# radoslawkrolikowski/financial-market-data-analysis

Measured on NVIDIA H100. Metric: sequences/sec (train step) biGRU h=256 seq=128 feat=64, higher is better.
Workload: dtype bf16x3 (fp32-class: split bf16 operand pairs on tensor cores, fp32 accumulate / state / gradients)

## Files before the change

financial_market_data_analysis_b200/csrc/tc_hopper.cuh:

```cuda
#pragma once
#include "common.cuh"
#include "kernels_f32.cuh"
#include <algorithm>
#include <map>
#include <mutex>
#include <cuda.h>
#include <cuda_bf16.h>

namespace htc {

typedef __nv_bfloat16 bf16_t;

__device__ __forceinline__ uint32_t smem_u32(const void* p) { return (uint32_t)__cvta_generic_to_shared(p); }

__device__ __forceinline__ void split_bf16(float x, bf16_t& hi, bf16_t& lo) {
    hi = __float2bfloat16(x);
    lo = __float2bfloat16(x - __bfloat162float(hi));
}

__device__ __forceinline__ void ldsm_x4(uint32_t addr, uint32_t (&r)[4]) {
    asm volatile("ldmatrix.sync.aligned.m8n8.x4.shared.b16 {%0, %1, %2, %3}, [%4];"
                 : "=r"(r[0]), "=r"(r[1]), "=r"(r[2]), "=r"(r[3]) : "r"(addr));
}
__device__ __forceinline__ void ldsm_x2(uint32_t addr, uint32_t (&r)[2]) {
    asm volatile("ldmatrix.sync.aligned.m8n8.x2.shared.b16 {%0, %1}, [%2];" : "=r"(r[0]), "=r"(r[1]) : "r"(addr));
}
__device__ __forceinline__ void mma_bf16(float (&c)[4], const uint32_t (&a)[4], uint32_t b0, uint32_t b1) {
    asm volatile("mma.sync.aligned.m16n8k16.row.col.f32.bf16.bf16.f32 {%0, %1, %2, %3}, {%4, %5, %6, %7}, {%8, %9}, "
                 "{%0, %1, %2, %3};"
                 : "+f"(c[0]), "+f"(c[1]), "+f"(c[2]), "+f"(c[3])
                 : "r"(a[0]), "r"(a[1]), "r"(a[2]), "r"(a[3]), "r"(b0), "r"(b1));
}

template <int PITCH>
__device__ __forceinline__ uint32_t swz(int row, int k) {
    return (uint32_t)(row * PITCH + ((((k >> 3) ^ (row & 7))) << 4) + ((k & 7) << 1));
}

__device__ __forceinline__ uint32_t mapa(uint32_t local_addr, uint32_t cta) {
    uint32_t r;
    asm volatile("mapa.shared::cluster.u32 %0, %1, %2;" : "=r"(r) : "r"(local_addr), "r"(cta));
    return r;
}
__device__ __forceinline__ void st_cluster_v2_f32(uint32_t addr, float2 v) {
    asm volatile("st.shared::cluster.v2.f32 [%0], {%1, %2};" ::"r"(addr), "f"(v.x), "f"(v.y) : "memory");
}
__device__ __forceinline__ void cluster_arrive() { asm volatile("barrier.cluster.arrive.release;" ::: "memory"); }
__device__ __forceinline__ void cluster_wait() { asm volatile("barrier.cluster.wait.acquire;" ::: "memory"); }
__device__ __forceinline__ uint32_t cluster_rank() {
    uint32_t r;
    asm volatile("mov.u32 %0, %%cluster_ctarank;" : "=r"(r));
    return r;
}

constexpr int WG_BM = 128, WG_BN = 128, WG_BK = 64;

__global__ void tc_pack_kernel(const float* __restrict__ src, int64_t s_r, int64_t s_k, int64_t zsrc, int R, int K, int Rp, int Kp,
                               bf16_t* __restrict__ hi, bf16_t* __restrict__ lo) {
    __shared__ float tile[32][33];
    const int z = blockIdx.z, r0 = blockIdx.y * 32, k0 = blockIdx.x * 32;
    const float* a = src + z * zsrc;
    const bool kfast = s_k == 1;
    for (int j = threadIdx.y; j < 32; j += 8) {
        const int r = r0 + (kfast ? j : threadIdx.x), k = k0 + (kfast ? threadIdx.x : j);
        float v = 0.f;
        if (r < R && k < K) v = a[(int64_t)r * s_r + (int64_t)k * s_k];
        if (kfast) tile[j][threadIdx.x] = v; else tile[threadIdx.x][j] = v;
    }
    __syncthreads();
    for (int j = threadIdx.y; j < 32; j += 8) {
        const int r = r0 + j, k = k0 + threadIdx.x;
        const int64_t o = ((int64_t)z * Rp + r) * Kp + k;
        bf16_t h, l;
        split_bf16(tile[j][threadIdx.x], h, l);
        hi[o] = h;
        if (lo) lo[o] = l;
    }
}

__global__ void to_planes_kernel(const float* __restrict__ src, int64_t rows, int cols, int pitch, bf16_t* __restrict__ hi,
                                 bf16_t* __restrict__ lo) {
    const int64_t n = rows * cols;
    for (int64_t i = (int64_t)blockIdx.x * blockDim.x + threadIdx.x; i < n; i += (int64_t)gridDim.x * blockDim.x) {
        const int64_t r = i / cols, c = i % cols, o = r * pitch + c;
        bf16_t h, l;
        split_bf16(src[i], h, l);
        hi[o] = h;
        if (lo) lo[o] = l;
    }
}

__device__ __forceinline__ void mbar_init(uint64_t* bar, uint32_t count) {
    asm volatile("mbarrier.init.shared::cta.b64 [%0], %1;" ::"r"(smem_u32(bar)), "r"(count) : "memory");
}
__device__ __forceinline__ void mbar_arrive_expect_tx(uint64_t* bar, uint32_t bytes) {
    asm volatile("mbarrier.arrive.expect_tx.shared::cta.b64 _, [%0], %1;" ::"r"(smem_u32(bar)), "r"(bytes) : "memory");
}
__device__ __forceinline__ void mbar_arrive(uint64_t* bar) {
    asm volatile("mbarrier.arrive.shared::cta.b64 _, [%0];" ::"r"(smem_u32(bar)) : "memory");
}
__device__ __forceinline__ bool mbar_try_wait(uint64_t* bar, uint32_t parity) {
    uint32_t ok;
    asm volatile(
        "{\n\t.reg .pred p;\n\t"
        "mbarrier.try_wait.parity.shared::cta.b64 p, [%1], %2;\n\t"
        "selp.u32 %0, 1, 0, p;\n\t}" : "=r"(ok) : "r"(smem_u32(bar)), "r"(parity) : "memory");
    return ok != 0;
}
__device__ __forceinline__ bool mbar_try_wait_cluster(uint64_t* bar, uint32_t parity) {
    uint32_t ok;
    asm volatile(
        "{\n\t.reg .pred p;\n\t"
        "mbarrier.try_wait.parity.acquire.cluster.shared::cta.b64 p, [%1], %2;\n\t"
        "selp.u32 %0, 1, 0, p;\n\t}" : "=r"(ok) : "r"(smem_u32(bar)), "r"(parity) : "memory");
    return ok != 0;
}
template <bool CLUSTER = false>
__device__ __forceinline__ void mbar_wait(uint64_t* bar, uint32_t parity) {
    auto ready = [&] { return CLUSTER ? mbar_try_wait_cluster(bar, parity) : mbar_try_wait(bar, parity); };
    if (ready()) return;
    uint64_t t0, t;
    asm volatile("mov.u64 %0, %%globaltimer;" : "=l"(t0));
    for (uint32_t i = 0;; ++i) {
        if (ready()) return;
        if ((i & 1023u) == 1023u) {
            asm volatile("mov.u64 %0, %%globaltimer;" : "=l"(t));
            if (t - t0 > 5000000000ull) __trap();
        }
    }
}
__device__ __forceinline__ void bulk_copy_to_peer(uint32_t src, uint32_t bytes, uint64_t* bar, uint32_t cta) {
    asm volatile("cp.async.bulk.shared::cluster.shared::cta.mbarrier::complete_tx::bytes [%0], [%1], %2, [%3];"
                 ::"r"(mapa(src, cta)), "r"(src), "r"(bytes), "r"(mapa(smem_u32(bar), cta)) : "memory");
}
__device__ __forceinline__ void tma_load_3d(uint32_t dst, const CUtensorMap* m, uint64_t* bar, int c0, int c1, int c2) {
    asm volatile("cp.async.bulk.tensor.3d.shared::cluster.global.mbarrier::complete_tx::bytes [%0], [%1, {%3, %4, %5}], [%2];"
                 ::"r"(dst), "l"(reinterpret_cast<uint64_t>(m)), "r"(smem_u32(bar)), "r"(c0), "r"(c1), "r"(c2) : "memory");
}
__device__ __forceinline__ uint64_t wg_desc(uint32_t saddr, uint32_t lbo) {
    return (uint64_t)((saddr & 0x3FFFF) >> 4) | ((uint64_t)(lbo >> 4) << 16) | ((uint64_t)(1024 >> 4) << 32) | ((uint64_t)1 << 62);
}
template <int TA, int TB>
__device__ __forceinline__ void wgmma_m64n128k16(float (&d)[64], uint64_t da, uint64_t db) {
    asm volatile("wgmma.mma_async.sync.aligned.m64n128k16.f32.bf16.bf16 {%0, %1, %2, %3, %4, %5, %6, %7, %8, %9, %10, %11, %12, %13, %14, %15, %16, %17, %18, %19, %20, %21, %22, %23, %24, %25, %26, %27, %28, %29, %30, %31, %32, %33, %34, %35, %36, %37, %38, %39, %40, %41, %42, %43, %44, %45, %46, %47, %48, %49, %50, %51, %52, %53, %54, %55, %56, %57, %58, %59, %60, %61, %62, %63}, %64, %65, 1, 1, 1, %66, %67;"
                 : "+f"(d[0]), "+f"(d[1]), "+f"(d[2]), "+f"(d[3]), "+f"(d[4]), "+f"(d[5]), "+f"(d[6]), "+f"(d[7]), "+f"(d[8]), "+f"(d[9]), "+f"(d[10]), "+f"(d[11]), "+f"(d[12]), "+f"(d[13]), "+f"(d[14]), "+f"(d[15]), "+f"(d[16]), "+f"(d[17]), "+f"(d[18]), "+f"(d[19]), "+f"(d[20]), "+f"(d[21]), "+f"(d[22]), "+f"(d[23]), "+f"(d[24]), "+f"(d[25]), "+f"(d[26]), "+f"(d[27]), "+f"(d[28]), "+f"(d[29]), "+f"(d[30]), "+f"(d[31]), "+f"(d[32]), "+f"(d[33]), "+f"(d[34]), "+f"(d[35]), "+f"(d[36]), "+f"(d[37]), "+f"(d[38]), "+f"(d[39]), "+f"(d[40]), "+f"(d[41]), "+f"(d[42]), "+f"(d[43]), "+f"(d[44]), "+f"(d[45]), "+f"(d[46]), "+f"(d[47]), "+f"(d[48]), "+f"(d[49]), "+f"(d[50]), "+f"(d[51]), "+f"(d[52]), "+f"(d[53]), "+f"(d[54]), "+f"(d[55]), "+f"(d[56]), "+f"(d[57]), "+f"(d[58]), "+f"(d[59]), "+f"(d[60]), "+f"(d[61]), "+f"(d[62]), "+f"(d[63])
                 : "l"(da), "l"(db), "n"(TA), "n"(TB));
}

struct WgOp {
    int zsel, coff, kshift[2];
};
struct WgJob {
    WgOp a, b;
    float* C; const float* bias; float* part;
    int M, N, tm, tn, batch, splits;
    int kblocks, kbd;
    int kcat;
    int beta;
    int64_t ldc, zC, zBias;
};

template <int NS, int STAGES, int AMN, int BMN>
__global__ void __launch_bounds__(384, 1)
wg_gemm_kernel(const __grid_constant__ CUtensorMap ta_hi, const __grid_constant__ CUtensorMap ta_lo,
               const __grid_constant__ CUtensorMap tb_hi, const __grid_constant__ CUtensorMap tb_lo, const WgJob j) {
    constexpr int NH = NS == 1 ? 1 : 2;
    constexpr int PLANE = WG_BM * WG_BK * 2;
    constexpr int STAGE = 2 * NH * PLANE;
    extern __shared__ __align__(1024) uint8_t wg_smem_raw[];
    uint8_t* sm = reinterpret_cast<uint8_t*>((reinterpret_cast<uintptr_t>(wg_smem_raw) + 1023) & ~(uintptr_t)1023);
    uint64_t* full = reinterpret_cast<uint64_t*>(sm + STAGES * STAGE);
    uint64_t* empty = full + STAGES;
    const int wgi = threadIdx.x / 128, tid = threadIdx.x % 128;
    const int units = j.tm * j.tn * j.batch * j.splits;
    const int per = (j.kblocks + j.splits - 1) / j.splits;
    if (threadIdx.x == 0) {
        for (int i = 0; i < STAGES; ++i) { mbar_init(full + i, 1); mbar_init(empty + i, 2); }
        asm volatile("fence.mbarrier_init.release.cluster;" ::: "memory");
    }
    __syncthreads();
    auto decode = [&](int u, int& s, int& zb, int& m0, int& n0) {
        s = u % j.splits; u /= j.splits;
        n0 = (u % j.tn) * WG_BN; u /= j.tn;
        m0 = (u % j.tm) * WG_BM; zb = u / j.tm;
    };

    if (wgi == 0) {
        if (tid == 0) {
            uint32_t it = 0;
            for (int u = blockIdx.x; u < units; u += gridDim.x) {
                int s, zb, m0, n0;
                decode(u, s, zb, m0, n0);
                const int kb1 = min(j.kblocks, (s + 1) * per);
                for (int kb = s * per; kb < kb1; ++kb, ++it) {
                    const int st = it % STAGES;
                    if (it >= STAGES) mbar_wait(empty + st, ((it / STAGES) - 1) & 1);
                    const uint32_t base = smem_u32(sm + st * STAGE);
                    mbar_arrive_expect_tx(full + st, STAGE);
                    const int dz = j.kcat ? kb / j.kbd : zb, kc = (j.kcat ? kb % j.kbd : kb) * WG_BK;
#pragma unroll
                    for (int h = 0; h < NH; ++h) {
                        const CUtensorMap* ma = h ? &ta_lo : &ta_hi;
                        const CUtensorMap* mb = h ? &tb_lo : &tb_hi;
                        const uint32_t da = base + h * PLANE, db = base + (NH + h) * PLANE;
                        if (AMN) {
                            const int k = kc + (dz ? j.a.kshift[1] : j.a.kshift[0]), r = m0 + dz * j.a.coff;
                            tma_load_3d(da, ma, full + st, r, k, dz * j.a.zsel);
                            tma_load_3d(da + PLANE / 2, ma, full + st, r + 64, k, dz * j.a.zsel);
                        } else {
                            tma_load_3d(da, ma, full + st, kc, m0, dz * j.a.zsel);
                        }
                        if (BMN) {
                            const int k = kc + (dz ? j.b.kshift[1] : j.b.kshift[0]), r = n0 + dz * j.b.coff;
                            tma_load_3d(db, mb, full + st, r, k, dz * j.b.zsel);
                            tma_load_3d(db + PLANE / 2, mb, full + st, r + 64, k, dz * j.b.zsel);
                        } else {
                            tma_load_3d(db, mb, full + st, kc, n0, dz * j.b.zsel);
                        }
                    }
                }
            }
        }
        return;
    }
    const int cg = wgi - 1;
    const int w = tid / 32, l = tid % 32;
    constexpr uint32_t AKS = AMN ? 2048 : 32, BKS = BMN ? 2048 : 32;
    constexpr uint32_t ALBO = AMN ? PLANE / 2 : 16, BLBO = BMN ? PLANE / 2 : 16;
    uint32_t it = 0;
    for (int u = blockIdx.x; u < units; u += gridDim.x) {
        int s, zb, m0, n0;
        decode(u, s, zb, m0, n0);
        const int kb1 = min(j.kblocks, (s + 1) * per);
        float d[64];
#pragma unroll
        for (int i = 0; i < 64; ++i) d[i] = 0.f;
        int prev = -1;
        for (int kb = s * per; kb < kb1; ++kb, ++it) {
            const int st = it % STAGES;
            mbar_wait(full + st, (it / STAGES) & 1);
            const uint32_t base = smem_u32(sm + st * STAGE);
            const uint32_t a_hi = base + cg * (PLANE / 2), a_lo = a_hi + PLANE;
            const uint32_t b_hi = base + NH * PLANE, b_lo = b_hi + PLANE;
            asm volatile("wgmma.fence.sync.aligned;" ::: "memory");
#pragma unroll
            for (int ks = 0; ks < WG_BK / 16; ++ks) {
                wgmma_m64n128k16<AMN, BMN>(d, wg_desc(a_hi + ks * AKS, ALBO), wg_desc(b_hi + ks * BKS, BLBO));
                if (NS != 1) {
                    wgmma_m64n128k16<AMN, BMN>(d, wg_desc(a_hi + ks * AKS, ALBO), wg_desc(b_lo + ks * BKS, BLBO));
                    wgmma_m64n128k16<AMN, BMN>(d, wg_desc(a_lo + ks * AKS, ALBO), wg_desc(b_hi + ks * BKS, BLBO));
                }
            }
            asm volatile("wgmma.commit_group.sync.aligned;" ::: "memory");
            asm volatile("wgmma.wait_group.sync.aligned 1;" ::: "memory");
            if (prev >= 0 && tid == 0) mbar_arrive(empty + prev);
            prev = st;
        }
        asm volatile("wgmma.wait_group.sync.aligned 0;" ::: "memory");
        if (prev >= 0 && tid == 0) mbar_arrive(empty + prev);
        float* C;
        int64_t ldc;
        const float* bias = nullptr;
        if (j.splits > 1) {
            C = j.part + ((int64_t)s * j.batch + zb) * j.M * j.N;
            ldc = j.N;
        } else {
            C = j.C + zb * j.zC;
            ldc = j.ldc;
            if (j.bias) bias = j.bias + zb * j.zBias;
        }
#pragma unroll
        for (int i = 0; i < 16; ++i)
#pragma unroll
            for (int e = 0; e < 4; ++e) {
                const int gm = m0 + cg * 64 + w * 16 + (l >> 2) + (e >= 2 ? 8 : 0);
                const int gn = n0 + 8 * i + 2 * (l & 3) + (e & 1);
                if (gm >= j.M || gn >= j.N) continue;
                float v = d[4 * i + e];
                if (bias) v += bias[gn];
                float* c = C + (int64_t)gm * ldc + gn;
                if (j.beta && j.splits == 1) *c += v;
                else *c = v;
            }
    }
}

__global__ void splitk_reduce_kernel(const float* __restrict__ part, int splits, int batch, int M, int N, float* __restrict__ C,
                                     int64_t ldc, int64_t zC, int beta) {
    const int64_t per = (int64_t)M * N, n = per * batch;
    for (int64_t i = (int64_t)blockIdx.x * blockDim.x + threadIdx.x; i < n; i += (int64_t)gridDim.x * blockDim.x) {
        float v = 0.f;
        for (int s = 0; s < splits; ++s) v += part[(int64_t)s * n + i];
        const int64_t z = i / per, r = i % per;
        float* c = C + z * zC + (r / N) * ldc + r % N;
        *c = beta ? *c + v : v;
    }
}

constexpr int SCAN_U = 64, SCAN_NB = 16, SCAN_THREADS = 256;
constexpr int SCAN_Y = 1, SCAN_G = 2, SCAN_PLANES = 4;
constexpr int SCAN_TRAIN = SCAN_Y | SCAN_G | SCAN_PLANES, SCAN_INFER_LOWER = SCAN_PLANES, SCAN_INFER_TOP = SCAN_Y;

template <int H, int NS>
struct FwdSmem {
    static constexpr int NH = NS == 1 ? 1 : 2;
    static constexpr int NBMAX = NS == 1 ? SCAN_NB : 2 * SCAN_NB;
    static constexpr int NBUF = NBMAX == SCAN_NB ? 2 : 1;
    static constexpr int WP = H * 2;
    static constexpr int WBYTES = 3 * SCAN_U * WP;
    static constexpr int HBYTES = NBMAX * H * 2;
    static constexpr int SLICE = NBMAX * SCAN_U * 2;
    static constexpr int TOTAL = NH * WBYTES + NBUF * NH * HBYTES + 2 * 8;
};

__device__ __forceinline__ void scan_tile(int q, int m2, int ntd, int D, int& d, int& bt0, int& nb) {
    if (q < D * m2) {
        d = q / m2; bt0 = (q % m2) * 2 * SCAN_NB; nb = 2 * SCAN_NB;
    } else {
        const int r = q - D * m2, o = ntd - 2 * m2;
        d = r / o; bt0 = (2 * m2 + r % o) * SCAN_NB; nb = SCAN_NB;
    }
}

template <int NBMAX>
__device__ __forceinline__ uint32_t hsw(int b, int k) {
    return (uint32_t)((k / SCAN_U) * (NBMAX * SCAN_U * 2)) + swz<SCAN_U * 2>(b, k % SCAN_U);
}

__device__ __forceinline__ void mbar_arrive_peer(uint64_t* bar, uint32_t cta) {
    asm volatile("mbarrier.arrive.release.cluster.shared::cluster.b64 _, [%0];" ::"r"(mapa(smem_u32(bar), cta)) : "memory");
}

template <int H, int NS, int OUT, bool LEN, int JN, bool RD = false>
__device__ __forceinline__ void gru_scan_fwd_tile(const float* __restrict__ gi, const float* __restrict__ Whh,
                                                  const float* __restrict__ bhh, int64_t zW, const float* __restrict__ h0,
                                                  float* __restrict__ Y, float* __restrict__ G, float* __restrict__ hn_out,
                                                  bf16_t* __restrict__ yh, bf16_t* __restrict__ yl, int B, int T, int D,
                                                  const int* __restrict__ lens, int d, int bt0,
                                                  const float* __restrict__ mask = nullptr) {
    using S = FwdSmem<H, NS>;
    constexpr int U = SCAN_U, CS = H / U, NH = S::NH, JMAX = JN, jn = JN, nb = JN * SCAN_NB;
    constexpr int NBMAX = nb, NBUF = S::NBUF * S::NBMAX / nb;
    constexpr int HBYTES = nb * H * 2, SLICE = nb * U * 2;
    static_assert(NBUF * HBYTES == S::NBUF * S::HBYTES, "both tile sizes fill the h region");
    static_assert(SCAN_THREADS % (nb * (U / 8)) == 0, "a thread copies the same Y plane row in every pass");
    extern __shared__ __align__(128) uint8_t smem[];
    uint8_t* Wsm = smem;
    uint8_t* Hsm = smem + NH * S::WBYTES;
    uint64_t* full = reinterpret_cast<uint64_t*>(Hsm + NBUF * NH * HBYTES);
    uint64_t* empty = full + 1;
    const int c = (int)cluster_rank();
    const int tid = threadIdx.x, lane = tid & 31, warp = tid >> 5;
    const float* W = Whh + d * zW;

    for (int i = tid; i < 3 * U * H; i += SCAN_THREADS) {
        const int q = i / H, k = i % H, gte = q / U, u = q % U;
        const float v = W[(int64_t)(gte * H + c * U + u) * H + k];
        bf16_t hi, lo;
        split_bf16(v, hi, lo);
        *reinterpret_cast<bf16_t*>(Wsm + swz<S::WP>(q, k)) = hi;
        if (NH == 2) *reinterpret_cast<bf16_t*>(Wsm + S::WBYTES + swz<S::WP>(q, k)) = lo;
    }
    for (int i = tid; i < nb * H; i += SCAN_THREADS) {
        const int b = i / H, k = i % H;
        float v = h0 ? h0[((int64_t)d * B + bt0 + b) * H + k] : 0.f;
        if constexpr (RD) v *= mask[((int64_t)d * B + bt0 + b) * H + k];
        bf16_t hi, lo;
        split_bf16(v, hi, lo);
        *reinterpret_cast<bf16_t*>(Hsm + hsw<NBMAX>(b, k)) = hi;
        if (NH == 2) *reinterpret_cast<bf16_t*>(Hsm + HBYTES + hsw<NBMAX>(b, k)) = lo;
    }
    if (tid == 0) {
        mbar_init(full, 1);
        mbar_init(full + 1, NBUF == 2 ? 1 : CS - 1);
        asm volatile("fence.mbarrier_init.release.cluster;" ::: "memory");
    }

    const int ug = warp >> 1, nt = warp & 1;
    int unit[2], bcol[JMAX][2];
    unit[0] = ug * 16 + (lane >> 2); unit[1] = unit[0] + 8;
#pragma unroll
    for (int j = 0; j < JMAX; ++j) {
        bcol[j][0] = (nt * jn + j) * 8 + 2 * (lane & 3); bcol[j][1] = bcol[j][0] + 1;
    }
    float bias[3][2], hp[JMAX][4], mk[RD ? JMAX : 1][4];
#pragma unroll
    for (int gte = 0; gte < 3; ++gte)
#pragma unroll
        for (int i = 0; i < 2; ++i) bias[gte][i] = bhh[d * zW + gte * H + c * U + unit[i]];
    int len[JMAX][2], rlen = T;
#pragma unroll
    for (int j = 0; j < JMAX; ++j) {
#pragma unroll
        for (int e = 0; e < 4; ++e) {
            const int b = bt0 + bcol[j][e & 1], k = c * U + unit[e >> 1];
            hp[j][e] = h0 ? h0[((int64_t)d * B + b) * H + k] : 0.f;
            if constexpr (RD) mk[j][e] = mask[((int64_t)d * B + b) * H + k];
        }
        len[j][0] = len[j][1] = T;
        if (LEN) { len[j][0] = lens[bt0 + bcol[j][0]]; len[j][1] = lens[bt0 + bcol[j][1]]; }
    }
    if (LEN) rlen = lens[bt0 + (tid / (U / 8)) % nb];
    cluster_arrive();
    cluster_wait();

    const int DH = D * H;
    for (int s = 0; s < T; ++s) {
        const int t = d == 0 ? s : T - 1 - s;
        const int buf = NBUF == 2 ? s & 1 : 0, nbuf = NBUF == 2 ? buf ^ 1 : 0;
        if (s > 0) mbar_wait<true>(full + buf, (NBUF == 2 ? (s - 1) >> 1 : s - 1) & 1);
        if (tid == 0 && s + 1 < T) mbar_arrive_expect_tx(full + nbuf, (CS - 1) * NH * nb * U * 2);
        float giv[3][JMAX][4];
#pragma unroll
        for (int j = 0; j < JMAX; ++j)
#pragma unroll
            for (int e = 0; e < 4; ++e) {
                const int64_t row = (int64_t)(bt0 + bcol[j][e & 1]) * T + t;
                const float* gr = gi + ((int64_t)d * B * T + row) * 3 * H + c * U + unit[e >> 1];
#pragma unroll
                for (int gte = 0; gte < 3; ++gte) giv[gte][j][e] = gr[gte * H];
            }
        float acc[3][JMAX][4];
#pragma unroll
        for (int gte = 0; gte < 3; ++gte)
#pragma unroll
            for (int j = 0; j < JMAX; ++j)
#pragma unroll
                for (int e = 0; e < 4; ++e) acc[gte][j][e] = 0.f;
        const uint32_t hbase = smem_u32(Hsm + buf * NH * HBYTES);
        const uint32_t wbase = smem_u32(Wsm);
#pragma unroll 4
        for (int ks = 0; ks < H / 16; ++ks) {
            uint32_t bh[JMAX][NH][2];
            const int bk = ks * 16 + ((lane >> 3) & 1) * 8;
#pragma unroll
            for (int j = 0; j < JMAX; ++j)
#pragma unroll
// ... 190 lines not shown
                if constexpr (RD) v = LEN && (d == 0 ? t + 1 : t - 1) >= plen[i] ? v : mk[i] * v;
                dhr[i] = v;
            }
        }
        cluster_arrive();
        __syncthreads();
#pragma unroll
        for (int i = 0; i < PAIRS; ++i) {
            const int p = tid + i * SCAN_THREADS, u = p % U, bl = p / U, b = bt0 + bl, j = c * U + u;
            const int64_t row = (int64_t)b * T + t;
            const float r = gr[i], z = gz[i], n = gn[i], hnv = ghn[i], hpv = hprev[i];
            const float dh = dhr[i] + dyv[i];
            float dan = dh * (1.f - z) * (1.f - n * n);
            float dar = dan * hnv * r * (1.f - r);
            float daz = dh * (hpv - n) * z * (1.f - z);
            float dgn = dan * r;
            const bool pad = LEN && t >= plen[i];
            if (pad) dan = dar = daz = dgn = 0.f;
            float* a = dgi + ((int64_t)d * B * T + row) * 3 * H + j;
            float* cg = dgh + ((int64_t)d * B * T + row) * 3 * H + j;
            a[0] = dar; a[H] = daz; a[2 * H] = dan;
            cg[0] = dar; cg[H] = daz; cg[2 * H] = dgn;
            dhz[i] = pad ? dhr[i] : dh * z;
            const float gv[3] = {dar, daz, dgn};
#pragma unroll
            for (int gte = 0; gte < 3; ++gte) {
                bf16_t hi, lo;
                split_bf16(gv[gte], hi, lo);
                *reinterpret_cast<bf16_t*>(Dsm + swz<S::WP>(bl, gte * U + u)) = hi;
                if (NH == 2) *reinterpret_cast<bf16_t*>(Dsm + S::DBYTES + swz<S::WP>(bl, gte * U + u)) = lo;
            }
            bf16_t hi, lo;
            split_bf16(dan, hi, lo);
            const int64_t po = ((int64_t)d * B * T + row) * 3 * H + 2 * H + j;
            gih[po] = hi;
            if (NH == 2) gil[po] = lo;
        }
        if (NS == 1 && s + 1 < T) load_step(s + 1);
        __syncthreads();
        for (int i = tid; i < NH * NR * (Q / 8); i += SCAN_THREADS) {
            const int h = i / (NR * Q / 8), r = (i / (Q / 8)) % NR, q = (i % (Q / 8)) * 8, gte = q / U;
            uint4 v = *reinterpret_cast<const uint4*>(Dsm + h * S::DBYTES + swz<S::WP>(r, q));
            const int64_t o = ((int64_t)d * B * T + (int64_t)(bt0 + r) * T + t) * 3 * H + gte * H + c * U + q % U;
            if (gte < 2) *reinterpret_cast<uint4*>((h ? gil : gih) + o) = v;
            if (first) v = make_uint4(0u, 0u, 0u, 0u);
            *reinterpret_cast<uint4*>((h ? ghl : ghh) + o) = v;
        }
        float acc[MT][2][4];
#pragma unroll
        for (int m = 0; m < MT; ++m)
#pragma unroll
            for (int n = 0; n < NBLK; ++n)
#pragma unroll
                for (int e = 0; e < 4; ++e) acc[m][n][e] = 0.f;
        const uint32_t wbase = smem_u32(Wsm), dbase = smem_u32(Dsm);
#pragma unroll 2
        for (int ks = 0; ks < Q / 16; ++ks) {
            uint32_t bv[NH][4];
            const int brow = (lane & 7) + ((lane >> 4) << 3), bk = ks * 16 + ((lane >> 3) & 1) * 8;
#pragma unroll
            for (int h = 0; h < NH; ++h) ldsm_x4(dbase + h * S::DBYTES + swz<S::WP>(brow, bk), bv[h]);
#pragma unroll
            for (int m = 0; m < MT; ++m) {
                const int arow = (warp + 8 * m) * 16 + (lane & 15), ak = ks * 16 + (lane >> 4) * 8;
                uint32_t a[NH][4];
#pragma unroll
                for (int h = 0; h < NH; ++h) ldsm_x4(wbase + h * S::WBYTES + swz<S::WP>(arow, ak), a[h]);
#pragma unroll
                for (int n = 0; n < NBLK; ++n) {
                    if (NS != 1) {
                        mma_bf16(acc[m][n], a[0], bv[NH - 1][2 * n], bv[NH - 1][2 * n + 1]);
                        mma_bf16(acc[m][n], a[NH - 1], bv[0][2 * n], bv[0][2 * n + 1]);
                    }
                    mma_bf16(acc[m][n], a[0], bv[0][2 * n], bv[0][2 * n + 1]);
                }
            }
        }
        if (NS != 1 && s + 1 < T) load_step(s + 1);
        __syncthreads();
        cluster_wait();
#pragma unroll
        for (int m = 0; m < MT; ++m)
#pragma unroll
            for (int n = 0; n < NBLK; ++n)
#pragma unroll
                for (int e = 0; e < 4; e += 2) {
                    const int k = (warp + 8 * m) * 16 + (lane >> 2) + (e >= 2 ? 8 : 0);
                    const int bl = n * 8 + 2 * (lane & 3);
                    const int dst = k / U, x = xslot(k % U, bl);
                    const float2 v = make_float2(acc[m][n][e], acc[m][n][e + 1]);
                    if (dst == c) {
                        *reinterpret_cast<float2*>(own + x) = v;
                    } else {
                        const float* rs = recv + (c < dst ? c : c - 1) * NB * U + x;
                        st_cluster_v2_f32(mapa(smem_u32(rs), dst), v);
                    }
                }
        cluster_arrive();
        cluster_wait();
    }
#pragma unroll
    for (int i = 0; i < PAIRS; ++i) {
        const int p = tid + i * SCAN_THREADS, u = p % U, b = p / U, x = xslot(u, b);
        float v = dhz[i];
#pragma unroll
        for (int src = 0; src < CS; ++src) v += slot(src)[x];
        if constexpr (RD) v = LEN && (d == 0 ? 0 : T - 1) >= plen[i] ? v : mk[i] * v;
        dhc[((int64_t)d * B + bt0 + b) * H + c * U + u] = v;
    }
}

template <int H, int NS, bool LEN, bool RD>
__global__ void __launch_bounds__(SCAN_THREADS, 1)
gru_scan_bwd_kernel(const float* __restrict__ G, const float* __restrict__ Y, const float* __restrict__ h0,
                    const float* __restrict__ dY, float* __restrict__ dhc, float* __restrict__ dgi, float* __restrict__ dgh,
                    const float* __restrict__ Whh, int64_t zW, bf16_t* __restrict__ gih, bf16_t* __restrict__ gil,
                    bf16_t* __restrict__ ghh, bf16_t* __restrict__ ghl, int B, int T, int D, int L8, const int* __restrict__ lens,
                    const float* __restrict__ mask) {
    const int ntd = B / SCAN_NB, n16 = D * ntd - L8, q = blockIdx.y;
    if (q < n16) {
        gru_scan_bwd_tile<H, NS, LEN, SCAN_NB, RD>(G, Y, h0, dY, dhc, dgi, dgh, Whh, zW, gih, gil, ghh, ghl, B, T, D, lens,
                                                    q / ntd, (q % ntd) * SCAN_NB, mask);
    } else {
        const int f = n16 + (q - n16) / 2;
        gru_scan_bwd_tile<H, NS, LEN, SCAN_NB / 2, RD>(G, Y, h0, dY, dhc, dgi, dgh, Whh, zW, gih, gil, ghh, ghl, B, T, D, lens,
                                                        f / ntd, (f % ntd) * SCAN_NB + ((q - n16) & 1) * (SCAN_NB / 2), mask);
    }
}

}

static inline int64_t rup(int64_t v, int64_t m) { return (v + m - 1) / m * m; }
static inline int64_t tc_pack_elems(int64_t R, int64_t K, int64_t batch, int prec) {
    return (prec == BIGRU_PREC_BF16X3 ? 2 : 1) * batch * rup(R, htc::WG_BM) * rup(K, htc::WG_BK);
}
static inline int64_t tc_gemm_ws_elems(int64_t M, int64_t N, int64_t K, int64_t batch, int prec) {
    return tc_pack_elems(M, K, batch, prec) + tc_pack_elems(N, K, batch, prec);
}
static inline int wg_splits(int64_t tiles, int64_t kblocks) {
    const int64_t s = std::min(cdiv64(4 * 132, tiles), kblocks / 8);
    if (s <= 1) return 1;
    const int64_t per = cdiv64(kblocks, s);
    return (int)cdiv64(kblocks, per);
}

struct Planes {
    const htc::bf16_t* hi; const htc::bf16_t* lo;
    int64_t cols, rows, depth, pitch;
};

typedef CUresult (*PFN_encodeTiled_t)(CUtensorMap*, CUtensorMapDataType, cuuint32_t, void*, const cuuint64_t*, const cuuint64_t*,
                                      const cuuint32_t*, const cuuint32_t*, CUtensorMapInterleave, CUtensorMapSwizzle,
                                      CUtensorMapL2promotion, CUtensorMapFloatOOBfill);
static int make_plane_map(CUtensorMap* m, const htc::bf16_t* base, const Planes& p, bool mn) {
    static PFN_encodeTiled_t enc = nullptr;
    if (!enc) {
        void* f = nullptr;
        cudaDriverEntryPointQueryResult q;
        if (cudaGetDriverEntryPoint("cuTensorMapEncodeTiled", &f, cudaEnableDefault, &q) != cudaSuccess || q != cudaDriverEntryPointSuccess) {
            bigru_set_error("tc_gemm: cuTensorMapEncodeTiled is unavailable");
            return BIGRU_ERR_CUDA;
        }
        enc = (PFN_encodeTiled_t)f;
    }
    const cuuint64_t dims[3] = {(cuuint64_t)p.cols, (cuuint64_t)p.rows, (cuuint64_t)p.depth};
    const cuuint64_t strides[2] = {(cuuint64_t)p.pitch * 2, (cuuint64_t)(p.pitch * p.rows) * 2};
    const cuuint32_t box[3] = {64u, mn ? 64u : 128u, 1u}, es[3] = {1u, 1u, 1u};
    CUresult r = enc(m, CU_TENSOR_MAP_DATA_TYPE_BFLOAT16, 3, const_cast<htc::bf16_t*>(base), dims, strides, box, es,
                     CU_TENSOR_MAP_INTERLEAVE_NONE, CU_TENSOR_MAP_SWIZZLE_128B, CU_TENSOR_MAP_L2_PROMOTION_L2_256B,
                     CU_TENSOR_MAP_FLOAT_OOB_FILL_NONE);
    if (r != CUDA_SUCCESS) { bigru_set_error("tc_gemm: cuTensorMapEncodeTiled failed (%d)", (int)r); return BIGRU_ERR_CUDA; }
    return BIGRU_OK;
}

template <int NS, int AMN, int BMN>
static int wg_launch(const CUtensorMap (&tm)[4], const htc::WgJob& j, int grid, cudaStream_t st) {
    constexpr int STAGES = NS == 1 ? 4 : 3;
    const int smem = STAGES * 2 * (NS == 1 ? 1 : 2) * 16384 + 1024 + 2 * STAGES * 8;
    auto k = htc::wg_gemm_kernel<NS, STAGES, AMN, BMN>;
    CUDA_TRY(cudaFuncSetAttribute(k, cudaFuncAttributeMaxDynamicSharedMemorySize, smem));
    k<<<grid, 384, smem, st>>>(tm[0], tm[1], tm[2], tm[3], j);
    LAUNCH_CHECK();
    return BIGRU_OK;
}

static int wg_gemm(htc::WgJob j, const Planes& A, bool amn, const Planes& B, bool bmn, int prec, cudaStream_t st) {
    if (j.M <= 0 || j.N <= 0) return BIGRU_OK;
    const bool x3 = prec == BIGRU_PREC_BF16X3;
    if (x3 != (A.lo != nullptr) || x3 != (B.lo != nullptr) || amn != bmn) {
        bigru_set_error("tc_gemm: operand planes do not match the precision / majors");
        return BIGRU_ERR_ARG;
    }
    j.tm = (int)cdiv64(j.M, htc::WG_BM);
    j.tn = (int)cdiv64(j.N, htc::WG_BN);
    CUtensorMap tm[4];
    TRY(make_plane_map(&tm[0], A.hi, A, amn));
    TRY(make_plane_map(&tm[2], B.hi, B, bmn));
    if (x3) {
        TRY(make_plane_map(&tm[1], A.lo, A, amn));
        TRY(make_plane_map(&tm[3], B.lo, B, bmn));
    } else {
        tm[1] = tm[0]; tm[3] = tm[2];
    }
    int dev = 0, nsm = 132;
    CUDA_TRY(cudaGetDevice(&dev));
    CUDA_TRY(cudaDeviceGetAttribute(&nsm, cudaDevAttrMultiProcessorCount, dev));
    const int64_t units = (int64_t)j.tm * j.tn * j.batch * j.splits;
    const int grid = (int)std::min<int64_t>(units, nsm);
    const int rc = amn ? (x3 ? wg_launch<3, 1, 1>(tm, j, grid, st) : wg_launch<1, 1, 1>(tm, j, grid, st))
                       : (x3 ? wg_launch<3, 0, 0>(tm, j, grid, st) : wg_launch<1, 0, 0>(tm, j, grid, st));
    TRY(rc);
    if (j.splits > 1) {
        const int64_t n = (int64_t)j.batch * j.M * j.N;
        htc::splitk_reduce_kernel<<<(unsigned)std::min<int64_t>(cdiv64(n, 256), 132 * 8), 256, 0, st>>>(j.part, j.splits, j.batch, j.M,
                                                                                                        j.N, j.C, j.ldc, j.zC, j.beta);
        LAUNCH_CHECK();
    }
    return BIGRU_OK;
}

static htc::WgJob wg_job(float* C, int M, int N, int64_t ldc, int batch, int64_t kblocks) {
    htc::WgJob j{};
    j.C = C; j.M = M; j.N = N; j.ldc = ldc; j.batch = batch; j.kblocks = (int)kblocks; j.kbd = (int)kblocks; j.splits = 1;
    return j;
}

static int tc_pack(const float* src, int64_t s_r, int64_t s_k, int64_t zsrc, int R, int K, int batch, int prec, htc::bf16_t* ws,
                   Planes* out, cudaStream_t st) {
    const bool x3 = prec == BIGRU_PREC_BF16X3;
    const int Rp = (int)rup(R, htc::WG_BM), Kp = (int)rup(K, htc::WG_BK);
    const int64_t sz = (int64_t)batch * Rp * Kp;
    *out = Planes{ws, x3 ? ws + sz : nullptr, Kp, Rp, batch, Kp};
    KLAUNCH(KC_PACK, 0.0, (4.0 + (x3 ? 4.0 : 2.0)) * batch * (double)R * K, st,
            htc::tc_pack_kernel<<<dim3(Kp / 32, Rp / 32, batch), dim3(32, 8), 0, st>>>(src, s_r, s_k, zsrc, R, K, Rp, Kp, ws,
                                                                                     x3 ? ws + sz : nullptr));
    return BIGRU_OK;
}

static int tc_gemm_launch(const GemmArgs& g, int prec, int cls, htc::bf16_t* ws, cudaStream_t st) {
    if (g.M <= 0 || g.N <= 0 || g.K <= 0) return BIGRU_OK;
    if (g.splitk != 1 || g.mask_period) {
        bigru_set_error("tc_gemm_launch: split-K and row masks are not supported");
        return BIGRU_ERR_ARG;
    }
    Planes A, B;
    TRY(tc_pack(g.A, g.sam, g.sak, g.zA, g.M, g.K, g.batch, prec, ws, &A, st));
    TRY(tc_pack(g.B, g.sbn, g.sbk, g.zB, g.N, g.K, g.batch, prec, ws + tc_pack_elems(g.M, g.K, g.batch, prec), &B, st));
    ProfScope ps(cls, 2.0 * g.M * g.N * (double)g.K * g.batch, 0.0, st);
    htc::WgJob j = wg_job(g.C, g.M, g.N, g.ldc, g.batch, cdiv64(g.K, htc::WG_BK));
    j.bias = g.bias; j.beta = g.beta; j.zC = g.zC; j.zBias = g.zBias;
    j.a.zsel = 1; j.b.zsel = 1;
    return wg_gemm(j, A, false, B, false, prec, st);
}

template <typename K>
static cudaLaunchConfig_t cluster_config(K kernel, int cs, int ny, int nz, int smem, cudaStream_t st, cudaLaunchAttribute* attr) {
    cudaLaunchConfig_t cfg{};
    cfg.gridDim = dim3(cs, ny, nz);
    cfg.blockDim = dim3(htc::SCAN_THREADS);
    cfg.dynamicSmemBytes = smem;
    cfg.stream = st;
    attr[0].id = cudaLaunchAttributeClusterDimension;
    attr[0].val.clusterDim.x = cs; attr[0].val.clusterDim.y = 1; attr[0].val.clusterDim.z = 1;
    cfg.attrs = attr; cfg.numAttrs = 1;
    return cfg;
}

template <typename... KArgs, typename... Args>
static int launch_cluster(void (*kernel)(KArgs...), int cs, int ny, int nz, int smem, cudaStream_t st, Args... args) {
    CUDA_TRY(cudaFuncSetAttribute(kernel, cudaFuncAttributeMaxDynamicSharedMemorySize, smem));
    cudaLaunchAttribute attr[1];
    const cudaLaunchConfig_t cfg = cluster_config(kernel, cs, ny, nz, smem, st, attr);
    CUDA_TRY(cudaLaunchKernelEx(&cfg, kernel, args...));
    return BIGRU_OK;
}

template <typename... KArgs>
static int cluster_residency(void (*kernel)(KArgs...), int cs, int smem, int* R) {
    static std::mutex mu;
    static std::map<std::pair<const void*, int>, int> cache;
    int dev = 0;
    CUDA_TRY(cudaGetDevice(&dev));
    const std::pair<const void*, int> key((const void*)kernel, dev);
    {
        std::lock_guard<std::mutex> g(mu);
        const auto it = cache.find(key);
        if (it != cache.end()) { *R = it->second; return BIGRU_OK; }
    }
    CUDA_TRY(cudaFuncSetAttribute(kernel, cudaFuncAttributeMaxDynamicSharedMemorySize, smem));
    cudaLaunchAttribute attr[1];
    const cudaLaunchConfig_t cfg = cluster_config(kernel, cs, 1, 1, smem, 0, attr);
    int n = 0;
    CUDA_TRY(cudaOccupancyMaxActiveClusters(&n, (void*)kernel, &cfg));
    if (n <= 0) { bigru_set_error("scan: no %d-CTA cluster with %d bytes of shared memory fits on this device", cs, smem); return BIGRU_ERR_DEVICE; }
    {
        std::lock_guard<std::mutex> g(mu);
        cache[key] = n;
    }
    *R = n;
    return BIGRU_OK;
}

static void scan_geometry(int R, bool two, int B, int D, int* m2, int* clusters) {
    const int ntd = B / htc::SCAN_NB, n = D * ntd;
    int n2 = 0;
    if (two) {
        const int rounds = (n + 2 * R - 1) / (2 * R);
        n2 = std::max(0, n - rounds * R);
        n2 = std::min((n2 + D - 1) / D * D, D * (ntd / 2));
    }
    *m2 = n2 / D;
    *clusters = n - n2;
}

static void scan_bwd_geometry(int R, int B, int D, int* L8, int* clusters) {
    const int n = D * (B / htc::SCAN_NB), rounds = (n + R - 1) / R, L = n - (rounds - 1) * R;
    *L8 = rounds > 1 && 2 * L <= R ? L : 0;
    *clusters = n + *L8;
}

typedef decltype(&htc::gru_scan_fwd_kernel<128, 1, htc::SCAN_TRAIN, false, false>) ScanFwdFn;
typedef decltype(&htc::gru_scan_bwd_kernel<128, 1, false, false>) ScanBwdFn;
struct ScanKernels {
    ScanFwdFn fwd; int fwd_smem; bool two;
    ScanBwdFn bwd; int bwd_smem;
};

template <int HH, int NS, bool LEN>
static ScanKernels scan_instance(int out, bool rd) {
    using namespace htc;
    const ScanFwdFn fwd = rd                        ? gru_scan_fwd_kernel<HH, NS, SCAN_TRAIN, LEN, true>
                          : out == SCAN_TRAIN       ? gru_scan_fwd_kernel<HH, NS, SCAN_TRAIN, LEN, false>
                          : out == SCAN_INFER_LOWER ? gru_scan_fwd_kernel<HH, NS, SCAN_INFER_LOWER, LEN, false>
                                                    : gru_scan_fwd_kernel<HH, NS, SCAN_INFER_TOP, LEN, false>;
    const ScanBwdFn bwd = rd ? gru_scan_bwd_kernel<HH, NS, LEN, true> : gru_scan_bwd_kernel<HH, NS, LEN, false>;
    return {fwd, FwdSmem<HH, NS>::TOTAL, FwdSmem<HH, NS>::NBMAX == 2 * SCAN_NB, bwd, BwdSmem<HH, NS>::TOTAL};
}

static int scan_kernels(const bigru_plan& p, int out, bool len, bool rd, ScanKernels* k) {
    using namespace htc;
    if (rd && out != SCAN_TRAIN) { bigru_set_error("tc_scan: recurrent dropout runs in the training forward only"); return BIGRU_ERR_ARG; }
    if (out != SCAN_TRAIN && out != SCAN_INFER_LOWER && out != SCAN_INFER_TOP) {
        bigru_set_error("tc_scan: no kernel writes this set of outputs (Y %d, G %d, planes %d)", (out & SCAN_Y) != 0,
                        (out & SCAN_G) != 0, (out & SCAN_PLANES) != 0);
        return BIGRU_ERR_ARG;
    }
    const bool x3 = p.prec == BIGRU_PREC_BF16X3;
    if (x3 && p.H == 128) *k = len ? scan_instance<128, 3, true>(out, rd) : scan_instance<128, 3, false>(out, rd);
    else if (x3 && p.H == 256) *k = len ? scan_instance<256, 3, true>(out, rd) : scan_instance<256, 3, false>(out, rd);
    else if (!x3 && p.H == 128) *k = len ? scan_instance<128, 1, true>(out, rd) : scan_instance<128, 1, false>(out, rd);
    else if (!x3 && p.H == 256) *k = len ? scan_instance<256, 1, true>(out, rd) : scan_instance<256, 1, false>(out, rd);
    else if (!x3 && p.H == 512) *k = len ? scan_instance<512, 1, true>(out, rd) : scan_instance<512, 1, false>(out, rd);
    else {
        bigru_set_error("tc_scan: no kernel for H=%d at precision %d", p.H, p.prec);
        return BIGRU_ERR_UNSUPPORTED;
    }
// ... 63 lines not shown
```

Baseline: 48320.

## Stage GEMM epilogue through swizzled shared memory and store C with TMA

Adds a TMA-based epilogue to the Hopper wgmma GEMM. Each consumer warpgroup writes its accumulators, with bias added, into 128B-swizzled fp32 staging boxes in shared memory and then issues bulk tensor stores, instead of scattered per-thread global writes. The aim is coalesced, asynchronous output writes that overlap with the next tile's mainloop. It enlarges the kernel's shared-memory footprint and adds named barriers, and it only applies when beta is zero or split-K is used and the output is 16-byte aligned.

```diff
diff --git a/financial_market_data_analysis_b200/csrc/tc_hopper.cuh b/financial_market_data_analysis_b200/csrc/tc_hopper.cuh
--- a/financial_market_data_analysis_b200/csrc/tc_hopper.cuh
+++ b/financial_market_data_analysis_b200/csrc/tc_hopper.cuh
@@ -54,6 +54,11 @@
 }
 
 constexpr int WG_BM = 128, WG_BN = 128, WG_BK = 64;
+constexpr int WG_CBOX = 64 * 32 * 4;
+__host__ __device__ constexpr int wg_cboxes(int ns) { return ns == 1 ? 4 : 2; }
+__host__ __device__ constexpr int wg_smem_bytes(int ns, int stages) {
+    return 1024 + stages * 2 * (ns == 1 ? 1 : 2) * WG_BM * WG_BK * 2 + 2 * wg_cboxes(ns) * WG_CBOX + 2 * stages * 8;
+}
 
 __global__ void tc_pack_kernel(const float* __restrict__ src, int64_t s_r, int64_t s_k, int64_t zsrc, int R, int K, int Rp, int Kp,
                                bf16_t* __restrict__ hi, bf16_t* __restrict__ lo) {
@@ -137,6 +142,15 @@
     asm volatile("cp.async.bulk.tensor.3d.shared::cluster.global.mbarrier::complete_tx::bytes [%0], [%1, {%3, %4, %5}], [%2];"
                  ::"r"(dst), "l"(reinterpret_cast<uint64_t>(m)), "r"(smem_u32(bar)), "r"(c0), "r"(c1), "r"(c2) : "memory");
 }
+__device__ __forceinline__ void tma_store_3d(const CUtensorMap* m, uint32_t src, int c0, int c1, int c2) {
+    asm volatile("cp.async.bulk.tensor.3d.global.shared::cta.bulk_group [%0, {%2, %3, %4}], [%1];"
+                 ::"l"(reinterpret_cast<uint64_t>(m)), "r"(src), "r"(c0), "r"(c1), "r"(c2) : "memory");
+}
+__device__ __forceinline__ void bulk_commit() { asm volatile("cp.async.bulk.commit_group;" ::: "memory"); }
+template <int N>
+__device__ __forceinline__ void bulk_wait_read() { asm volatile("cp.async.bulk.wait_group.read %0;" ::"n"(N) : "memory"); }
+__device__ __forceinline__ void bulk_wait_all() { asm volatile("cp.async.bulk.wait_group 0;" ::: "memory"); }
+__device__ __forceinline__ void named_sync(int id, int n) { asm volatile("bar.sync %0, %1;" ::"r"(id), "r"(n) : "memory"); }
 __device__ __forceinline__ uint64_t wg_desc(uint32_t saddr, uint32_t lbo) {
     return (uint64_t)((saddr & 0x3FFFF) >> 4) | ((uint64_t)(lbo >> 4) << 16) | ((uint64_t)(1024 >> 4) << 32) | ((uint64_t)1 << 62);
 }
@@ -157,19 +171,22 @@
     int kblocks, kbd;
     int kcat;
     int beta;
+    int cmap;
     int64_t ldc, zC, zBias;
 };
 
 template <int NS, int STAGES, int AMN, int BMN>
 __global__ void __launch_bounds__(384, 1)
 wg_gemm_kernel(const __grid_constant__ CUtensorMap ta_hi, const __grid_constant__ CUtensorMap ta_lo,
-               const __grid_constant__ CUtensorMap tb_hi, const __grid_constant__ CUtensorMap tb_lo, const WgJob j) {
+               const __grid_constant__ CUtensorMap tb_hi, const __grid_constant__ CUtensorMap tb_lo,
+               const __grid_constant__ CUtensorMap tc, const WgJob j) {
     constexpr int NH = NS == 1 ? 1 : 2;
     constexpr int PLANE = WG_BM * WG_BK * 2;
     constexpr int STAGE = 2 * NH * PLANE;
+    constexpr int CB = wg_cboxes(NS);
     extern __shared__ __align__(1024) uint8_t wg_smem_raw[];
     uint8_t* sm = reinterpret_cast<uint8_t*>((reinterpret_cast<uintptr_t>(wg_smem_raw) + 1023) & ~(uintptr_t)1023);
-    uint64_t* full = reinterpret_cast<uint64_t*>(sm + STAGES * STAGE);
+    uint64_t* full = reinterpret_cast<uint64_t*>(sm + STAGES * STAGE + 2 * CB * WG_CBOX);
     uint64_t* empty = full + STAGES;
     const int wgi = threadIdx.x / 128, tid = threadIdx.x % 128;
     const int units = j.tm * j.tn * j.batch * j.splits;
@@ -258,6 +275,44 @@
         }
         asm volatile("wgmma.wait_group.sync.aligned 0;" ::: "memory");
         if (prev >= 0 && tid == 0) mbar_arrive(empty + prev);
+        if (j.cmap) {
+            const float* bias = j.splits == 1 && j.bias ? j.bias + zb * j.zBias : nullptr;
+            const int zc = j.splits > 1 ? s * j.batch + zb : zb;
+            const int q = l & 3, r8 = l >> 2;
+            float bv[32];
+#pragma unroll
+            for (int i = 0; i < 16; ++i)
+#pragma unroll
+                for (int e = 0; e < 2; ++e) {
+                    const int gn = n0 + 8 * i + 2 * q + e;
+                    bv[2 * i + e] = bias && gn < j.N ? bias[gn] : 0.f;
+                }
+            uint8_t* stg = sm + STAGES * STAGE + cg * CB * WG_CBOX;
+#pragma unroll
+            for (int c = 0; c < 4; ++c) {
+                const uint32_t box = smem_u32(stg + (c % CB) * WG_CBOX);
+                if (tid == 0) bulk_wait_read<CB - 1>();
+                named_sync(1 + cg, 128);
+#pragma unroll
+                for (int ii = 0; ii < 4; ++ii) {
+                    const int i = 4 * c + ii;
+#pragma unroll
+                    for (int h = 0; h < 2; ++h) {
+                        float v0 = d[4 * i + 2 * h], v1 = d[4 * i + 2 * h + 1];
+                        if (bias) { v0 += bv[2 * i]; v1 += bv[2 * i + 1]; }
+                        const uint32_t a = box + (w * 16 + r8 + 8 * h) * 128 + (((2 * ii + (q >> 1)) ^ r8) << 4) + (q & 1) * 8;
+                        asm volatile("st.shared.v2.f32 [%0], {%1, %2};" ::"r"(a), "f"(v0), "f"(v1) : "memory");
+                    }
+                }
+                asm volatile("fence.proxy.async.shared::cta;" ::: "memory");
+                named_sync(1 + cg, 128);
+                if (tid == 0) {
+                    if (n0 + 32 * c < j.N) tma_store_3d(&tc, box, n0 + 32 * c, m0 + cg * 64, zc);
+                    bulk_commit();
+                }
+            }
+            continue;
+        }
         float* C;
         int64_t ldc;
         const float* bias = nullptr;
@@ -283,6 +338,7 @@
                 else *c = v;
             }
     }
+    if (j.cmap && tid == 0) bulk_wait_all();
 }
 
 __global__ void splitk_reduce_kernel(const float* __restrict__ part, int splits, int batch, int M, int N, float* __restrict__ C,
@@ -779,7 +835,8 @@
 typedef CUresult (*PFN_encodeTiled_t)(CUtensorMap*, CUtensorMapDataType, cuuint32_t, void*, const cuuint64_t*, const cuuint64_t*,
                                       const cuuint32_t*, const cuuint32_t*, CUtensorMapInterleave, CUtensorMapSwizzle,
                                       CUtensorMapL2promotion, CUtensorMapFloatOOBfill);
-static int make_plane_map(CUtensorMap* m, const htc::bf16_t* base, const Planes& p, bool mn) {
+static int encode_map(CUtensorMap* m, CUtensorMapDataType type, int esize, const void* base, int64_t cols, int64_t rows,
+                      int64_t depth, int64_t pitch, int64_t zstride, uint32_t box0, uint32_t box1) {
     static PFN_encodeTiled_t enc = nullptr;
     if (!enc) {
         void* f = nullptr;
@@ -790,23 +847,28 @@
         }
         enc = (PFN_encodeTiled_t)f;
     }
-    const cuuint64_t dims[3] = {(cuuint64_t)p.cols, (cuuint64_t)p.rows, (cuuint64_t)p.depth};
-    const cuuint64_t strides[2] = {(cuuint64_t)p.pitch * 2, (cuuint64_t)(p.pitch * p.rows) * 2};
-    const cuuint32_t box[3] = {64u, mn ? 64u : 128u, 1u}, es[3] = {1u, 1u, 1u};
-    CUresult r = enc(m, CU_TENSOR_MAP_DATA_TYPE_BFLOAT16, 3, const_cast<htc::bf16_t*>(base), dims, strides, box, es,
-                     CU_TENSOR_MAP_INTERLEAVE_NONE, CU_TENSOR_MAP_SWIZZLE_128B, CU_TENSOR_MAP_L2_PROMOTION_L2_256B,
-                     CU_TENSOR_MAP_FLOAT_OOB_FILL_NONE);
+    const cuuint64_t dims[3] = {(cuuint64_t)cols, (cuuint64_t)rows, (cuuint64_t)depth};
+    const cuuint64_t strides[2] = {(cuuint64_t)(pitch * esize), (cuuint64_t)(zstride * esize)};
+    const cuuint32_t box[3] = {box0, box1, 1u}, es[3] = {1u, 1u, 1u};
+    CUresult r = enc(m, type, 3, const_cast<void*>(base), dims, strides, box, es, CU_TENSOR_MAP_INTERLEAVE_NONE,
+                     CU_TENSOR_MAP_SWIZZLE_128B, CU_TENSOR_MAP_L2_PROMOTION_L2_256B, CU_TENSOR_MAP_FLOAT_OOB_FILL_NONE);
     if (r != CUDA_SUCCESS) { bigru_set_error("tc_gemm: cuTensorMapEncodeTiled failed (%d)", (int)r); return BIGRU_ERR_CUDA; }
     return BIGRU_OK;
 }
 
+static int make_plane_map(CUtensorMap* m, const htc::bf16_t* base, const Planes& p, bool mn) {
+    return encode_map(m, CU_TENSOR_MAP_DATA_TYPE_BFLOAT16, 2, base, p.cols, p.rows, p.depth, p.pitch, p.pitch * p.rows, 64u,
+                      mn ? 64u : 128u);
+}
+
 template <int NS, int AMN, int BMN>
-static int wg_launch(const CUtensorMap (&tm)[4], const htc::WgJob& j, int grid, cudaStream_t st) {
+static int wg_launch(const CUtensorMap (&tm)[5], const htc::WgJob& j, int grid, cudaStream_t st) {
     constexpr int STAGES = NS == 1 ? 4 : 3;
-    const int smem = STAGES * 2 * (NS == 1 ? 1 : 2) * 16384 + 1024 + 2 * STAGES * 8;
+    constexpr int smem = htc::wg_smem_bytes(NS, STAGES);
+    static_assert(smem <= 232448, "wg_gemm_kernel: more shared memory than an sm_90 block may have");
     auto k = htc::wg_gemm_kernel<NS, STAGES, AMN, BMN>;
     CUDA_TRY(cudaFuncSetAttribute(k, cudaFuncAttributeMaxDynamicSharedMemorySize, smem));
-    k<<<grid, 384, smem, st>>>(tm[0], tm[1], tm[2], tm[3], j);
+    k<<<grid, 384, smem, st>>>(tm[0], tm[1], tm[2], tm[3], tm[4], j);
     LAUNCH_CHECK();
     return BIGRU_OK;
 }
@@ -820,7 +882,7 @@
     }
     j.tm = (int)cdiv64(j.M, htc::WG_BM);
     j.tn = (int)cdiv64(j.N, htc::WG_BN);
-    CUtensorMap tm[4];
+    CUtensorMap tm[5];
     TRY(make_plane_map(&tm[0], A.hi, A, amn));
     TRY(make_plane_map(&tm[2], B.hi, B, bmn));
     if (x3) {
@@ -829,6 +891,13 @@
     } else {
         tm[1] = tm[0]; tm[3] = tm[2];
     }
+    const bool split = j.splits > 1;
+    float* const cbase = split ? j.part : j.C;
+    const int64_t depth = split ? (int64_t)j.splits * j.batch : j.batch, ldc = split ? j.N : j.ldc;
+    const int64_t zc = depth == 1 ? j.M * ldc : split ? (int64_t)j.M * j.N : j.zC;
+    j.cmap = (split || !j.beta) && reinterpret_cast<uintptr_t>(cbase) % 16 == 0 && ldc % 4 == 0 && zc % 4 == 0;
+    if (j.cmap) TRY(encode_map(&tm[4], CU_TENSOR_MAP_DATA_TYPE_FLOAT32, 4, cbase, j.N, j.M, depth, ldc, zc, 32u, 64u));
+    else tm[4] = tm[0];
     int dev = 0, nsm = 132;
     CUDA_TRY(cudaGetDevice(&dev));
     CUDA_TRY(cudaDeviceGetAttribute(&nsm, cudaDevAttrMultiProcessorCount, dev));
```

Result: faster. 51870 (median of 6 runs) (+7.3%).
